# lucastrefezza/quadruplet-sentence-transformer

Hardware: AMD Instinct MI355X
Metric: quadruplets/sec (seq_len=128, all-MiniLM-L6-v2) training step (higher is better)
Workload: dtype bf16; 1 GPU; all-MiniLM-L6-v2 dims (random-init), 64 quadruplets/GPU x 1 GPU, seq_len=128, fwd + gamma-quadruplet loss + bwd + clip + AdamW, dropout 0.1 on hidden states and attention probabilities as the reference's train() mode (BASELINE.json configs[1]); global_batch=64, seq_len=128, parallelism=dp1, precision=bf16 MFMA operands, fp32 accumulate/residual/LN/softmax/loss/optimizer, launch=eager

## Files before the change

### include/qst.h

```cpp
#ifndef QST_H
#define QST_H

#include <stddef.h>
#include <stdint.h>

#ifdef __cplusplus
extern "C" {
#endif

typedef enum {
    QST_OK = 0,
    QST_ERR_BAD_ARG = -1,
    QST_ERR_UNSUPPORTED = -2,
    QST_ERR_WORKSPACE = -3,
    QST_ERR_HIP = -4,
    QST_ERR_NO_DEVICE = -5,
    QST_ERR_COMM = -6,
    QST_ERR_NO_FORWARD = -7
} qst_status;

enum { QST_ARCH_BERT = 0, QST_ARCH_MPNET = 1, QST_ARCH_ROBERTA = 2 };
enum { QST_PREC_BF16 = 0, QST_PREC_BF16X3 = 1, QST_PREC_FP8 = 3, QST_PREC_F16 = 4, QST_PREC_F16W = 5 };
enum { QST_REDUCE_NONE = 0, QST_REDUCE_SUM = 1, QST_REDUCE_MEAN = 2 };

// ... 16 lines not shown

typedef struct qst_encoder qst_encoder;

const char* qst_strerror(int status);
int  qst_last_hip_error(void);
int  qst_version(void);

int64_t qst_arena_elems(const qst_config* cfg);
int     qst_arena_num_segments(const qst_config* cfg);
int     qst_arena_segment(const qst_config* cfg, int idx, const char** name_out, int64_t* offset_out,
                          int64_t* numel_out, int32_t* decay_out, int32_t* gemm_out);
int64_t qst_shadow_elems(const qst_config* cfg);

int64_t qst_shadow8_bytes(const qst_config* cfg);

int  qst_encoder_create(const qst_config* cfg, qst_encoder** out);
void qst_encoder_destroy(qst_encoder* enc);

size_t qst_encoder_saved_bytes(const qst_encoder* enc, int nseq, int L, int training);
size_t qst_encoder_bwd_workspace_bytes(const qst_encoder* enc, int nseq, int L);

int qst_refresh_shadow(const qst_encoder* enc, const float* params, void* shadow_bf16, void* stream);
int qst_refresh_shadow_mx(const qst_encoder* enc, const float* params, void* shadow_mx, void* stream);

int qst_encoder_forward(qst_encoder* enc, const int64_t* ids, const int64_t* mask, const int64_t* type_ids,
                        int nseq, int L, const float* params, const void* shadow_bf16,
                        float* out_emb, float* out_tok, void* saved, size_t saved_bytes, int training,
                        void* stream);

int qst_encoder_set_dropout(qst_encoder* enc, float p_hidden, float p_attn, uint32_t* state_dev);
int qst_dropout_init(uint32_t* state_dev, uint64_t seed, void* stream);
int qst_encoder_set_ffn_chain(qst_encoder* enc, int mask);
int qst_encoder_set_ln_fusion(qst_encoder* enc, int mode);
#define QST_POOL_CLS 1
#define QST_POOL_MAX 2
#define QST_POOL_MEAN 4
#define QST_POOL_MEAN_SQRT 8
#define QST_POOL_WMEAN 16
#define QST_POOL_ALL 31
int qst_encoder_set_pooling(qst_encoder* enc, int mode);
int qst_encoder_embedding_dim(const qst_encoder* enc);
int qst_dropout_advance(uint32_t* state_dev, void* stream);

int qst_encoder_backward(qst_encoder* enc, const int64_t* ids, const int64_t* mask, const int64_t* type_ids,
                         int nseq, int L, const float* params, const void* shadow_bf16,
                         const float* grad_emb, float* grads, void* saved, size_t saved_bytes,
                         void* workspace, size_t workspace_bytes, void* stream);

int qst_encoder_backward_partial(qst_encoder* enc, const int64_t* ids, const int64_t* mask, const int64_t* type_ids,
                                 int nseq, int L, const float* params, const void* shadow_bf16,
                                 const float* grad_emb, float* grads, void* saved, size_t saved_bytes,
                                 void* workspace, size_t workspace_bytes,
                                 int do_head, int layer_hi, int layer_lo, int do_embed, void* stream);

enum { QST_BWD_HEAD = 1, QST_BWD_EMBED = 2, QST_BWD_SKIP_WGRAD = 4, QST_BWD_WGRAD_ONLY = 8 };
int qst_encoder_backward_stage(qst_encoder* enc, const int64_t* ids, const int64_t* mask, const int64_t* type_ids,
                               int nseq, int L, const float* params, const void* shadow_bf16,
                               const float* grad_emb, float* grads, void* saved, size_t saved_bytes,
                               void* workspace, size_t workspace_bytes,
                               int flags, int layer_hi, int layer_lo, void* stream);

int qst_quadruplet_loss(const float* xa, const float* xp, const float* xq, const float* xn,
                        int B, int D, float gamma, float margin_pos_neg, float margin_pos_part,
                        float margin_part_neg, float p, int swap, int reduction,
                        float* out_loss, const float* grad_out,
                        float* grad_a, float* grad_p, float* grad_q, float* grad_n,
// ... 120 lines not shown
```

### quadruplet-sentence-transformer_amd/_lib.py

```python
from __future__ import annotations

import ctypes as C
import os
from typing import Optional

_HERE = os.path.dirname(os.path.abspath(__file__))
LIB_PATH = os.path.join(_HERE, "libqst.so")

c_i64p = C.POINTER(C.c_int64)
c_i32p = C.POINTER(C.c_int32)
c_f32p = C.POINTER(C.c_float)
vp = C.c_void_p


class QstError(RuntimeError):
    pass


class QstConfig(C.Structure):
    _fields_ = [("arch", C.c_int32), ("vocab_size", C.c_int32), ("hidden_size", C.c_int32),
                ("num_layers", C.c_int32), ("num_heads", C.c_int32), ("intermediate_size", C.c_int32),
                ("max_position", C.c_int32), ("type_vocab_size", C.c_int32), ("layer_norm_eps", C.c_float),
                ("normalize", C.c_int32), ("rel_buckets", C.c_int32), ("rel_max_distance", C.c_int32),
                ("pad_token_id", C.c_int32), ("precision", C.c_int32)]
# ... 123 lines not shown
    "qst_gemm_nt8_f8": (C.c_int, [C.POINTER(QstGemmArgs), C.c_int, C.c_int, vp]),
    "qst_gemm8_mode": (C.c_int, [C.c_int]),
    "qst_embed_ln_fwd": (C.c_int, [vp, vp, vp, vp, vp, vp, vp, vp, C.c_float, C.c_int, C.c_int, vp, vp, vp, vp, vp]),
    "qst_embed_ln_fwd_drop": (C.c_int, [vp, vp, vp, vp, vp, vp, vp, vp, C.c_float, C.c_int, C.c_int, vp, vp, vp, vp,
                                        C.POINTER(QstDrop), vp]),
    "qst_ln_fwd_mx": (C.c_int, [vp, vp, vp, C.c_float, C.c_int, C.c_int, vp, vp, vp, vp, vp]),
    "qst_embed_ln_fwd_mx": (C.c_int, [vp, vp, vp, vp, vp, vp, vp, vp, C.c_float, C.c_int, C.c_int, vp, vp, vp, vp, vp]),
    "qst_ln_fwd_mx_train": (C.c_int, [vp, vp, vp, C.c_float, C.c_int, C.c_int, vp, vp, vp, vp, vp, vp, vp]),
    "qst_embed_ln_fwd_mx_train": (C.c_int, [vp, vp, vp, vp, vp, vp, vp, vp, C.c_float, C.c_int, C.c_int, vp, vp, vp, vp, vp, vp,
                                            vp, vp]),
    "qst_ln_fwd": (C.c_int, [vp, vp, vp, C.c_float, C.c_int, C.c_int, vp, vp, vp, vp, vp]),
    "qst_ln_bwd_scratch_bytes": (C.c_size_t, [C.c_int, C.c_int]),
    "qst_ln_bwd_reduce_batch": (C.c_int, [vp, vp]),
    "qst_ln_bwd": (C.c_int, [vp, vp, vp, vp, C.c_int, C.c_int, vp, vp, vp, vp, vp, vp]),
    "qst_ln_bwd_drop": (C.c_int, [vp, vp, vp, vp, C.c_int, C.c_int, vp, vp, vp, vp, vp, C.POINTER(QstDrop), C.POINTER(QstDrop), vp]),
    "qst_embed_bwd": (C.c_int, [vp, vp, vp, vp, C.c_int, C.c_int, C.c_int, C.c_int, vp, vp, vp, vp]),
    "qst_position_ids": (C.c_int, [vp, C.c_int, C.c_int, C.c_int, C.c_int, vp, vp]),
    "qst_forward_prologue": (C.c_int, [vp, C.c_int, C.c_int, C.c_int, C.c_int, vp, vp, vp, vp]),
    "qst_pool_fwd": (C.c_int, [vp, vp, C.c_int, C.c_int, C.c_int, C.c_int, C.c_int, vp, vp, vp, vp]),
    "qst_pool_bwd": (C.c_int, [vp, vp, vp, vp, C.c_int, C.c_int, C.c_int, C.c_int, C.c_int, vp, vp]),
    "qst_attention_fwd": (C.c_int, [vp, vp, vp, C.c_int, C.c_int, C.c_int, C.c_int, vp, vp, vp]),
    "qst_attention_bwd": (C.c_int, [vp, vp, vp, vp, vp, vp, C.c_int, C.c_int, C.c_int, C.c_int, vp, vp, vp, vp]),
    "qst_attention_fwd_ex": (C.c_int, [C.POINTER(QstAttnDesc), vp]),
    "qst_attention_bwd_ex": (C.c_int, [C.POINTER(QstAttnDesc), vp]),
    "qst_dropout_multipliers": (C.c_int, [C.POINTER(QstDrop), C.c_int, C.c_int64, vp, vp]),
    "qst_abi_sizeof": (C.c_int64, [C.c_int]),
    "qst_normalize_rows": (C.c_int, [vp, C.c_int, C.c_int, vp, vp]),
    "qst_cls_head_fwd": (C.c_int, [vp, C.c_int64, C.c_int, C.c_int, vp, vp, vp, vp, C.c_int, C.c_int, C.c_int, vp, vp]),
    "qst_dropout_init": (C.c_int, [vp, C.c_uint64, vp]),
    "qst_dropout_advance": (C.c_int, [vp, vp]),
    "qst_encoder_set_dropout": (C.c_int, [vp, C.c_float, C.c_float, vp]),
    "qst_encoder_set_ffn_chain": (C.c_int, [vp, C.c_int]),
    "qst_encoder_set_ln_fusion": (C.c_int, [vp, C.c_int]),
    "qst_encoder_set_pooling": (C.c_int, [vp, C.c_int]),
    "qst_encoder_embedding_dim": (C.c_int, [vp]),
    "qst_transpose_f32": (C.c_int, [vp, C.c_int, C.c_int, C.c_int, vp, C.c_int, vp]),
    "qst_gelu_f32": (C.c_int, [vp, C.c_int64, vp, vp]),
    "qst_gelu_bwd_f32": (C.c_int, [vp, vp, C.c_int64, vp, vp]),
    "qst_colsum_f32": (C.c_int, [vp, C.c_int, C.c_int, C.c_int, vp, vp]),
    "qst_embed_sum_f32": (C.c_int, [vp, vp, vp, vp, vp, vp, C.c_int, C.c_int, vp, vp]),
    "qst_ln_bwd_f32": (C.c_int, [vp, vp, vp, C.c_float, C.c_int, C.c_int, vp, vp, vp, vp]),
    "qst_attention_bwd_f32": (C.c_int, [vp, vp, vp, vp, vp, C.c_int, C.c_int, C.c_int, C.c_int, vp, vp, vp]),
    "qst_attention_bwd_f32_drop": (C.c_int, [vp, vp, vp, vp, vp, C.c_int, C.c_int, C.c_int, C.c_int, vp, vp, vp, vp]),
    "qst_attention_bwd_x3_scratch_bytes": (C.c_size_t, [C.c_int, C.c_int, C.c_int]),
    "qst_attention_bwd_x3": (C.c_int, [vp, vp, vp, vp, vp, C.c_int, C.c_int, C.c_int, C.c_int, vp, vp, vp, vp, vp]),
    "qst_dropout_apply_f32": (C.c_int, [vp, vp, vp, C.c_int64, vp, vp]),
    "qst_comm_unique_id": (C.c_int, [vp]),
    "qst_comm_init": (C.c_int, [C.c_int, C.c_int, vp, C.POINTER(vp)]),
    "qst_allreduce_bucket": (C.c_int, [vp, vp, C.c_int64, C.c_int, vp]),
    "qst_comm_rank": (C.c_int, [vp]),
    "qst_comm_world": (C.c_int, [vp]),
    "qst_comm_destroy": (None, [vp]),
    "qst_comm_last_error": (C.c_char_p, []),
    "qst_rel_bucket_host": (C.c_int, [C.c_int, C.c_int, C.c_int]),
    "qst_rel_bias_fwd": (C.c_int, [vp, vp, C.c_int, C.c_int, vp, vp]),
    "qst_rel_bias_bwd": (C.c_int, [vp, vp, C.c_int, C.c_int, C.c_int, vp, vp]),
    "qst_rel_pos_fwd": (C.c_int, [vp, vp, C.c_int, C.c_int, vp, vp]),
    "qst_rel_pos_bwd": (C.c_int, [vp, vp, C.c_int, C.c_int, C.c_int, vp, vp]),
    "qst_topk_rows": (C.c_int, [vp, C.c_int64, vp, C.c_int, C.c_int, C.c_int, vp, vp, vp]),
    "qst_topk_merge_rows": (C.c_int, [vp, C.c_int64, C.c_int, C.c_int, C.c_int64, C.c_int64, C.c_int, C.c_float, C.c_int,
                                      vp, vp, vp]),
    "qst_topk_stream_workspace_bytes": (C.c_size_t, [C.c_int, C.c_int, C.c_int]),
    "qst_topk_stream": (C.c_int, [vp, vp, C.c_int, C.c_int, C.c_int, C.c_int, C.c_int, C.c_int, C.c_int64, C.c_int64,
                                  C.c_int, C.c_float, vp, vp, vp, C.c_size_t, vp]),
    "qst_community_workspace_bytes": (C.c_size_t, [C.c_int, C.c_int, C.c_int]),
    "qst_community_count": (C.c_int, [vp, C.c_int, C.c_int, C.c_float, C.c_int, vp, vp, vp, C.c_size_t, vp]),
# ... 70 lines not shown
```

### quadruplet-sentence-transformer_amd/csrc/qst_api.hip

```cpp
#include <math.h>
#include <stdio.h>
#include <string.h>
#include <string>
#include <vector>
#include <mutex>
#include <unordered_map>
#include <algorithm>

#include "qst_common.h"
#include "qst_kernels.h"

static thread_local int g_last_hip_error = 0;
extern "C" int qst_set_hip_error(int code) { g_last_hip_error = code; return code; }
extern "C" int qst_last_hip_error(void) { return g_last_hip_error; }
extern "C" int qst_version(void) { return 114; }

extern "C" const char* qst_strerror(int s) {
    switch (s) {
        case QST_OK: return "ok";
        case QST_ERR_BAD_ARG: return "bad argument (null pointer, non-positive size or bad enum)";
        case QST_ERR_UNSUPPORTED: return "unsupported dimensions for the gfx950 kernels";
        case QST_ERR_WORKSPACE: return "workspace or saved-activation arena too small";
        case QST_ERR_HIP: return "HIP runtime error (see qst_last_hip_error)";
        case QST_ERR_NO_DEVICE: return "no HIP device";
        case QST_ERR_COMM: return "RCCL error (see qst_comm_last_error)";
        case QST_ERR_NO_FORWARD: return "no matching training forward: `saved` is not an activation arena that a training forward of this "
                                        "precision and shape (nseq, L) has filled in this process";
        default: return "unknown qst status";
    }
}

namespace {

constexpr int64_t kAlign = 256;

struct Seg {
    std::string name;
    int64_t off, numel;
    int rows, cols;
    int decay, gemm;
    int64_t shadow_off;
};

struct Layout {
    std::vector<Seg> segs;
    int64_t total = 0, shadow_total = 0;
    int word = -1, pos = -1, type = -1, eg = -1, eb = -1, rel = -1;
    std::vector<int> layer0;
// ... 57 lines not shown
uint64_t g_rec_seq = 0;
void rec_put(const void* saved, uint32_t hidden, uint32_t attn, int kind, int nseq, int L, int pool) {
    std::lock_guard<std::mutex> lk(g_rec_mu);
    g_recs[saved] = FwdRec{hidden, attn, kind, ++g_rec_seq, nseq, L, pool};
    if (g_recs.size() > 4096) {
        std::vector<uint64_t> seqs;
        seqs.reserve(g_recs.size());
        for (const auto& kv : g_recs) seqs.push_back(kv.second.seq);
        std::nth_element(seqs.begin(), seqs.end() - 2048, seqs.end());
        const uint64_t cut = *(seqs.end() - 2048);
        for (auto it = g_recs.begin(); it != g_recs.end();) it = it->second.seq < cut ? g_recs.erase(it) : std::next(it);
    }
}
bool rec_get(const void* saved, int kind, int nseq, int L, FwdRec* out) {
    std::lock_guard<std::mutex> lk(g_rec_mu);
    const auto it = g_recs.find(saved);
    if (it == g_recs.end() || it->second.kind != kind || it->second.nseq != nseq || it->second.L != L) return false;
    *out = it->second;
    return true;
}
}

struct qst_encoder {
    qst_config cfg;
    Layout lay;
    uint8_t* chunk_decay = nullptr;
    int32_t* rel_lut = nullptr;
    int64_t* shadow_tab = nullptr;
    int shadow_nseg = 0, shadow_blocks = 0;
    uint32_t drop_hidden = 0, drop_attn = 0;
    uint32_t* drop_state = nullptr;
    int ffn_chain = 1;
    int ln_fusion = 0;
    int pool = QST_POOL_MEAN;
};

extern "C" int64_t qst_arena_elems(const qst_config* cfg) { return cfg_ok(cfg) ? build_layout(cfg).total : QST_ERR_BAD_ARG; }
extern "C" int64_t qst_shadow_elems(const qst_config* cfg) {
    if (!cfg_ok(cfg)) return QST_ERR_BAD_ARG;
    const int64_t n = build_layout(cfg).shadow_total;
    return cfg->precision == QST_PREC_F16W ? 2 * n : n;
}
extern "C" int64_t qst_shadow8_bytes(const qst_config* cfg) { return cfg_ok(cfg) ? build_layout(cfg).shadow_total : QST_ERR_BAD_ARG; }
extern "C" int qst_arena_num_segments(const qst_config* cfg) { return cfg_ok(cfg) ? (int)build_layout(cfg).segs.size() : QST_ERR_BAD_ARG; }
extern "C" int qst_arena_segment(const qst_config* cfg, int idx, const char** name_out, int64_t* offset_out,
                                 int64_t* numel_out, int32_t* decay_out, int32_t* gemm_out) {
    if (!cfg_ok(cfg)) return QST_ERR_BAD_ARG;
    static thread_local Layout L;
    L = build_layout(cfg);
    if (idx < 0 || idx >= (int)L.segs.size()) return QST_ERR_BAD_ARG;
    const Seg& s = L.segs[idx];
    if (name_out) *name_out = s.name.c_str();
    if (offset_out) *offset_out = s.off;
    if (numel_out) *numel_out = s.numel;
    if (decay_out) *decay_out = s.decay;
    if (gemm_out) *gemm_out = s.gemm;
    return QST_OK;
}

extern "C" int qst_rel_bucket_host(int rel , int num_buckets, int max_distance) {
    int n = -rel;
    const int nb = num_buckets / 2;
    int ret = (n < 0) ? nb : 0;
    n = n < 0 ? -n : n;
    const int max_exact = nb / 2;
    if (n < max_exact) return ret + n;
// ... 168 lines not shown
    return p;
}

struct MxPlan { size_t pos_ids, x[2], xb, xq, xs, qkv, ctx, cq, cs, s, y1, y1b, yq, ys, hq, hs, pooled, rel, argmax, total; };
MxPlan plan_mx(const qst_config& c, int nseq, int L, int pool) {
    MxPlan p;
    const size_t M = (size_t)nseq * L, H = c.hidden_size, I = c.intermediate_size, A = c.num_heads;
    Bump take;
    p.pos_ids = take(M * 4);
    p.x[0] = take(M * H * 4); p.x[1] = take(M * H * 4);
    p.xb = take(M * H * 2); p.xq = take(M * H); p.xs = take(M * H / 32);
    p.qkv = take(M * 3 * H * 2); p.ctx = take(M * H * 2); p.cq = take(M * H); p.cs = take(M * H / 32);
    p.s = take(M * H * 4); p.y1 = take(M * H * 4); p.y1b = take(M * H * 2); p.yq = take(M * H); p.ys = take(M * H / 32);
    p.hq = take(M * I); p.hs = take(M * I / 32);
    p.pooled = take((size_t)nseq * pool_dim(c, pool) * 4);
    p.rel = (c.arch == QST_ARCH_MPNET) ? take(A * (size_t)2 * L * 4) : 0;
    p.argmax = take_argmax(take, c, nseq, pool);
    p.total = take.off;
    return p;
}
struct MxOperands { size_t xq, xs, cq, cs, yq, ys, hq, hs, total; };
MxOperands plan_mx_train_operands(const qst_config& c, int nseq, int L, size_t base) {
    MxOperands t;
    const size_t M = (size_t)nseq * L, H = c.hidden_size, I = c.intermediate_size;
    Bump take{base};
    t.xq = take(M * H); t.xs = take(M * H / 32);
    t.cq = take(M * H); t.cs = take(M * H / 32);
    t.yq = take(M * H); t.ys = take(M * H / 32);
    t.hq = take(M * I); t.hs = take(M * I / 32);
    t.total = take.off;
    return t;
}

struct BwdPlan { size_t dxa, dxb, ds, dsb, dsb1, du, dctx, dqkv, drel, lnred, lnred_stride, delta, total; };
BwdPlan plan_bwd(const qst_config& c, int nseq, int L) {
    BwdPlan p;
    const size_t M = (size_t)nseq * L, H = c.hidden_size, I = c.intermediate_size, A = c.num_heads;
    Bump take;
    p.dxa = take(M * H * 4); p.dxb = take(M * H * 4); p.ds = take(M * H * 4); p.dsb = take(M * H * 2);
    p.dsb1 = take(M * H * 2);
    p.du = take(M * I * 2); p.dctx = take(M * H * 2); p.dqkv = take(M * 3 * H * 2);
    p.drel = (c.arch == QST_ARCH_MPNET) ? take(A * (size_t)2 * L * 4) : 0;
    p.lnred_stride = (qst_ln_bwd_scratch_bytes((int)M, (int)H) + 255) / 256 * 256;
    p.lnred = take(p.lnred_stride * (size_t)(2 * c.num_layers + 1));
    p.delta = take((size_t)nseq * A * L * 4);
    p.total = take.off;
    return p;
}

int shape_ok(const qst_encoder* e, int nseq, int L) {
    if (!e || nseq <= 0 || L <= 0) return QST_ERR_BAD_ARG;
    if (L % 32 != 0 || L > 512) return QST_ERR_UNSUPPORTED;
    if ((int64_t)nseq * L * e->cfg.intermediate_size * 2 >= ((int64_t)1 << 32)) return QST_ERR_UNSUPPORTED;
    if (e->cfg.arch == QST_ARCH_BERT && L > e->cfg.max_position) return QST_ERR_UNSUPPORTED;
    if (e->cfg.arch != QST_ARCH_BERT && L + e->cfg.pad_token_id + 1 > e->cfg.max_position) return QST_ERR_UNSUPPORTED;
    return QST_OK;
}

}

extern "C" int qst_encoder_set_ffn_chain(qst_encoder* e, int mask) {
    if (!e || mask < 0 || mask > 7) return QST_ERR_BAD_ARG;
    e->ffn_chain = mask;
    return QST_OK;
}
extern "C" int qst_encoder_set_ln_fusion(qst_encoder* e, int mode) {
    if (!e || mode < 0 || mode > 2) return QST_ERR_BAD_ARG;
    e->ln_fusion = mode;
    return QST_OK;
}
extern "C" int qst_encoder_set_pooling(qst_encoder* e, int mode) {
    if (!e || mode < 0 || mode > QST_POOL_ALL) return QST_ERR_BAD_ARG;
    e->pool = mode ? mode : QST_POOL_MEAN;
    return QST_OK;
}
extern "C" int qst_encoder_embedding_dim(const qst_encoder* e) {
    return e ? (int)pool_dim(e->cfg, e->pool) : QST_ERR_BAD_ARG;
}
extern "C" int qst_encoder_set_dropout(qst_encoder* e, float p_hidden, float p_attn, uint32_t* state_dev) {
    if (!e || !(p_hidden >= 0.f && p_hidden < 1.f) || !(p_attn >= 0.f && p_attn < 1.f)) return QST_ERR_BAD_ARG;
    if ((p_hidden > 0.f || p_attn > 0.f) && !state_dev) return QST_ERR_BAD_ARG;
    auto thr = [](float p) { const long t = lroundf(p * 65536.f); return (uint32_t)(t > 65535 ? 65535 : t); };
    e->drop_hidden = thr(p_hidden); e->drop_attn = thr(p_attn);
    e->drop_state = (e->drop_hidden || e->drop_attn) ? state_dev : nullptr;
    return QST_OK;
}

extern "C" size_t qst_encoder_saved_bytes(const qst_encoder* e, int nseq, int L, int training) {
    if (shape_ok(e, nseq, L) != QST_OK) return 0;
    const int pool = e->pool;
    if (e->cfg.precision == QST_PREC_BF16X3)
        return training ? plan_x3_train(e->cfg, nseq, L, pool).total : plan_x3(e->cfg, nseq, L, pool).total;
    if (e->cfg.precision == QST_PREC_FP8)
        return training ? plan_mx_train_operands(e->cfg, nseq, L, plan_acts(e->cfg, nseq, L, true, pool).total).total
                        : plan_mx(e->cfg, nseq, L, pool).total;
    return plan_acts(e->cfg, nseq, L, training != 0, pool).total;
}
extern "C" size_t qst_encoder_bwd_workspace_bytes(const qst_encoder* e, int nseq, int L) {
    if (shape_ok(e, nseq, L) != QST_OK) return 0;
    if (e->cfg.precision == QST_PREC_BF16X3) return plan_x3_bwd(e->cfg, nseq, L).total;
    return plan_bwd(e->cfg, nseq, L).total;
}

namespace {

struct OpKernels {
    decltype(&qst_gemm_nt) gemm_nt;
    decltype(&qst_gemm_nt_ln) gemm_nt_ln;
    decltype(&qst_ffn_chain) ffn_chain;
    decltype(&qst_gemm_tn_group) gemm_tn_group;
    decltype(&qst_embed_ln_fwd_drop) embed_ln_fwd_drop;
    decltype(&qst_ln_fwd) ln_fwd;
    decltype(&qst_ln_bwd_drop) ln_bwd_drop;
    decltype(&qst_attention_fwd_ex) attention_fwd_ex;
    decltype(&qst_attention_bwd_ex) attention_bwd_ex;
    decltype(&qst_shadow_all) shadow_all;
    int arena_kind;
};
const OpKernels kOpBf16 = {qst_gemm_nt, qst_gemm_nt_ln, qst_ffn_chain, qst_gemm_tn_group, qst_embed_ln_fwd_drop, qst_ln_fwd,
                           qst_ln_bwd_drop, qst_attention_fwd_ex, qst_attention_bwd_ex, qst_shadow_all, ARENA_BF16};
const OpKernels kOpF16 = {qst_gemm_nt_f16, qst_gemm_nt_ln_f16, qst_ffn_chain_f16, qst_gemm_tn_group_f16,
                          qst_embed_ln_fwd_drop_f16, qst_ln_fwd_f16, qst_ln_bwd_drop_f16, qst_attention_fwd_ex_f16,
                          qst_attention_bwd_ex_f16, qst_shadow_all_f16, ARENA_F16};
const OpKernels& op_kernels(const qst_config& c) {
    return (c.precision == QST_PREC_F16 || c.precision == QST_PREC_F16W) ? kOpF16 : kOpBf16;
}

constexpr int kFuseLnMinRows = 16384;
static bool fuse_ln_rows(int H, int M, int mode) {
    if (!qst_gemm_nt_ln_supported(H) || mode == 2) return false;
    if (mode == 1) return true;
    if (qst_gemm_nt_ln_block_rows(H) == 128) return M >= kFuseLnMinRows;
    return (int64_t)((M + 255) / 256) * (H / 256) >= 512 || (H % 384 == 0 && (int64_t)((M + 127) / 128) * (H / 384) >= 512);
}
// ... 360 lines not shown
        const int b = lay.layer0[l];
        const X3Layer& a = p.layers[l];
        const float* xin = l == 0 ? F(p.x0) : F(p.layers[l - 1].x);
        QST_TRY(qst_ln_bwd_f32(dx, F(a.s2), P(b + LN2_G), eps, M, H, ds, G(b + LN2_G), G(b + LN2_B), st));
        const float* dsm = ds;
        QST_TRY(masked(ds, QST_DROP_SITE_FFN_OUT(l), dctx, &dsm));
        QST_TRY(qst_transpose_f32(P(b + W_2), H, I, I, wT, H, st));
        QST_TRY(nt3(dsm, wT, dbig, I, H, 5, {.aux = F(a.u)}));
        QST_TRY(wgrad(dsm, H, F(a.h), I, b + W_2, b + B_2));
        QST_TRY(dgrad(dbig, I, b + W_1, H, dy, ds));
        QST_TRY(wgrad(dbig, I, F(a.y1), H, b + W_1, b + B_1));
        QST_TRY(qst_ln_bwd_f32(dy, F(a.s1), P(b + LN1_G), eps, M, H, ds, G(b + LN1_G), G(b + LN1_B), st));
        QST_TRY(masked(ds, QST_DROP_SITE_ATTN_OUT(l), dy, &dsm));
        QST_TRY(dgrad(dsm, H, b + W_O, H, dctx, nullptr));
        QST_TRY(wgrad(dsm, H, F(a.ctx), H, b + W_O, b + B_O));
        const QstDrop dp = probs(QST_DROP_SITE_PROBS(l));
        QST_TRY(qst_attention_bwd_x3(F(a.qkv), F(a.ctx), dctx, mask, rel, nseq, L, A, d, dqkv, drel, ws + w.astats, &dp, st));
        QST_TRY(dgrad(dqkv, 3 * H, b + W_QKV, H, dx, ds));
        QST_TRY(wgrad(dqkv, 3 * H, xin, H, b + W_QKV, b + B_QKV));
    }
    if (!(flags & QST_BWD_EMBED)) return QST_OK;
    const QstDrop de = hidden(QST_DROP_SITE_EMBED);
    if (de.state) QST_TRY(qst_dropout_apply_f32(&de, dx, nullptr, (int64_t)M * H, dx, st));
    QST_TRY(qst_ln_bwd_f32(dx, F(p.s0), P(lay.eg), eps, M, H, ds, G(lay.eg), G(lay.eb), st));
    QST_TRY(qst_embed_bwd(ds, ids, type_ids, (const int32_t*)(sv + p.pos_ids), nseq, L, H, c.type_vocab_size,
                          G(lay.word), G(lay.pos), G(lay.type), st));
    if (c.arch == QST_ARCH_MPNET) QST_TRY(qst_rel_bias_bwd(drel, e->rel_lut, c.rel_buckets, A, L, G(lay.rel), st));
    return QST_OK;
}

int Pass::backward_op16(const void* shadow, const float* grad_emb, size_t saved_bytes, size_t workspace_bytes, int flags,
                        int layer_hi, int layer_lo) {
    const ActPlan p = plan_acts(c, nseq, L, true, e->pool);
    const BwdPlan w = plan_bwd(c, nseq, L);
    if (saved_bytes < p.total || workspace_bytes < w.total) return QST_ERR_WORKSPACE;
    const uint16_t* sh = (const uint16_t*)shadow;
    auto WT = [&](int seg) { return sh + lay.segs[seg].shadow_off + qst_align_up(lay.segs[seg].numel, kAlign); };

    float* dxa = (float*)(ws + w.dxa);
    float* dxb = (float*)(ws + w.dxb);
    float* ds = (float*)(ws + w.ds);
    void* dsb = ws + w.dsb;
    void* dsb1 = ws + w.dsb1;
    void* du = ws + w.du;
    void* dctx = ws + w.dctx;
    void* dqkv = ws + w.dqkv;
    QstLnReduceBatch lnb{};
    lnb.H = H;
    lnb.nblocks = (int)(qst_ln_bwd_scratch_bytes(M, H) / ((size_t)2 * H * sizeof(float)));
    const bool fuse_ln = fuse_ln_rows(H, M, e->ln_fusion);
    QST_TRY(backward_dropout(ops.arena_kind, p.dropst));
    const bool fuse_ffn = fuse_ln && !dropping && (e->ffn_chain & 4) && qst_ffn_chain_supported(H, I) != 0;
    const int fused_rows = (M + qst_gemm_nt_ln_block_rows_m(H, M) - 1) / qst_gemm_nt_ln_block_rows_m(H, M);
    auto ln_slot = [&](int slot, float* dg, float* db, int nrows = 0) {
        float* sp = (float*)(ws + w.lnred + (size_t)slot * w.lnred_stride);
        lnb.partials[lnb.count] = sp; lnb.dgamma[lnb.count] = dg; lnb.dbeta[lnb.count] = db;
        lnb.nblocks_each[lnb.count] = nrows;
        ++lnb.count;
        return sp;
    };
    float* drel = nullptr;
    if (c.arch == QST_ARCH_MPNET) {
        drel = (float*)(ws + w.drel);
        rel = F(p.rel);
        if (flags & QST_BWD_HEAD) QST_HIP_CHECK(hipMemsetAsync(drel, 0, (size_t)A * 2 * L * 4, st));
    }
    if (flags & QST_BWD_HEAD) QST_TRY(head_bwd(grad_emb, p.pooled, p.argmax, dxa));
    auto wgrad = [&](int l) -> int {
        const LayerAct& a = p.layers[l];
        const int b = lay.layer0[l];
        const void* xin_b = (l == 0) ? (const void*)(sv + p.x0b) : (const void*)(sv + p.layers[l - 1].xb);
        QstTnGroup grp{};
        grp.nprob = 4;
        grp.splits = 0;
        auto set = [&](int i, const void* dY, int N, const void* X, int K, int wseg, int bseg) {
            QstGemmArgs& q = grp.prob[i];
            q.A = dY; q.B = X; q.C = G(wseg); q.colsum = G(bseg); q.M = M; q.N = N; q.K = K;
            q.lda = N; q.ldb = K; q.ldc = K;
        };
        set(0, dsb, H, sv + a.hact, I, b + W_2, b + B_2);
        set(1, du, I, sv + a.y1b, H, b + W_1, b + B_1);
        set(2, dsb1, H, sv + a.ctx, H, b + W_O, b + B_O);
        set(3, dqkv, 3 * H, xin_b, H, b + W_QKV, b + B_QKV);
        return ops.gemm_tn_group(&grp, st);
    };
    if (flags & QST_BWD_WGRAD_ONLY) return wgrad(layer_lo);
    for (int l = layer_hi - 1; l >= layer_lo; --l) {
        const LayerAct& a = p.layers[l];
        const int b = lay.layer0[l];
        if (!fuse_ln || l == c.num_layers - 1)
            QST_TRY(ops.ln_bwd_drop(dxa, sv + a.xh2, F(a.rs2), P(b + LN2_G), M, H, ds, dsb, nullptr, nullptr,
                                    ln_slot(2 * l + 1, G(b + LN2_G), G(b + LN2_B)), nullptr,
                                    active(hidden(QST_DROP_SITE_FFN_OUT(l))), st));
        if (!fuse_ffn) QST_TRY(nt(dsb, WT(b + W_2), du, I, H, QST_EPI_GELU_BWD, {.aux = sv + a.u}));
        const float* ds1 = ds;
        const QstDrop d1 = hidden(QST_DROP_SITE_ATTN_OUT(l));
        if (fuse_ffn) {
            QST_TRY(ffn({.A = dsb, .B1 = WT(b + W_2), .B2 = WT(b + W_1), .resid = ds, .aux = sv + a.u, .save_h = du, .C = dxb,
                         .C2 = dsb1},
                        1, {.gamma = P(b + LN1_G), .xhat = sv + a.xh1, .rstd = F(a.rs1),
                            .partials = ln_slot(2 * l, G(b + LN1_G), G(b + LN1_B), fused_rows)}));
            ds1 = dxb;
        } else if (fuse_ln) {
            QST_TRY(nt_ln(du, WT(b + W_1), dxb, I, 1, {.C2 = dsb1, .resid = ds, .drop = d1, .drop_where = 2},
                          {.gamma = P(b + LN1_G), .xhat = sv + a.xh1, .rstd = F(a.rs1),
                           .partials = ln_slot(2 * l, G(b + LN1_G), G(b + LN1_B), fused_rows)}));
            ds1 = dxb;
        } else {
            QST_TRY(nt(du, WT(b + W_1), dxb, H, I, QST_EPI_F32_RESID, {.resid = ds}));
            QST_TRY(ops.ln_bwd_drop(dxb, sv + a.xh1, F(a.rs1), P(b + LN1_G), M, H, ds, dsb1, nullptr, nullptr,
                                    ln_slot(2 * l, G(b + LN1_G), G(b + LN1_B)), nullptr, active(d1), st));
        }
        QST_TRY(nt(dsb1, WT(b + W_O), dctx, H, H, QST_EPI_BF16));
        QstAttnDesc q = attn(l, sv + a.qkv, sv + a.ctx, F(a.lse));
        q.dctx = dctx; q.dqkv = dqkv; q.drel = drel; q.delta_scratch = (float*)(ws + w.delta);
        QST_TRY(ops.attention_bwd_ex(&q, st));
        if (!(flags & QST_BWD_SKIP_WGRAD)) QST_TRY(wgrad(l));
        if (fuse_ln && l > 0) {
            const LayerAct& lo = p.layers[l - 1];
            const int bl = lay.layer0[l - 1];
            QST_TRY(nt_ln(dqkv, WT(b + W_QKV), ds, 3 * H, 1,
                          {.C2 = dsb, .resid = ds1, .drop = hidden(QST_DROP_SITE_FFN_OUT(l - 1)), .drop_where = 2},
                          {.gamma = P(bl + LN2_G), .xhat = sv + lo.xh2, .rstd = F(lo.rs2),
                           .partials = ln_slot(2 * (l - 1) + 1, G(bl + LN2_G), G(bl + LN2_B), fused_rows)}));
        } else if (fuse_ln) {
            QST_TRY(nt_ln(dqkv, WT(b + W_QKV), ds, 3 * H, 1, {.resid = ds1, .drop = hidden(QST_DROP_SITE_EMBED), .drop_where = 3},
                          {.gamma = P(lay.eg), .xhat = sv + p.xh0, .rstd = F(p.rs0),
                           .partials = ln_slot(2 * c.num_layers, G(lay.eg), G(lay.eb), fused_rows)}));
        } else {
            QST_TRY(nt(dqkv, WT(b + W_QKV), dxa, H, 3 * H, QST_EPI_F32_RESID, {.resid = ds1}));
        }
    }
    const bool do_embed = (flags & QST_BWD_EMBED) != 0;
    if (do_embed && !fuse_ln)
        QST_TRY(ops.ln_bwd_drop(dxa, sv + p.xh0, F(p.rs0), P(lay.eg), M, H, ds, nullptr, nullptr, nullptr,
                                ln_slot(2 * c.num_layers, G(lay.eg), G(lay.eb)), active(hidden(QST_DROP_SITE_EMBED)), nullptr, st));
    if (lnb.count > 0) {
        if (lnb.count > QST_LN_BATCH_MAX) return QST_ERR_UNSUPPORTED;
        QST_TRY(qst_ln_bwd_reduce_batch(&lnb, st));
    }
    if (!do_embed) return QST_OK;
    QST_TRY(qst_embed_bwd(ds, ids, type_ids, (const int32_t*)(sv + p.pos_ids), nseq, L, H, c.type_vocab_size,
                          G(lay.word), G(lay.pos), G(lay.type), st));
    if (c.arch == QST_ARCH_MPNET) QST_TRY(qst_rel_pos_bwd(drel, e->rel_lut, c.rel_buckets, A, L, G(lay.rel), st));
    return QST_OK;
}

}

extern "C" int qst_refresh_shadow(const qst_encoder* e, const float* params, void* shadow, void* stream) {
    if (!e || !params || !shadow) return QST_ERR_BAD_ARG;
    if (e->cfg.precision == QST_PREC_F16W)
        return qst_shadow_all_split_f16(params, shadow, (uint16_t*)shadow + e->lay.shadow_total, e->shadow_tab, e->shadow_nseg,
                                        e->shadow_blocks, stream);
    return op_kernels(e->cfg).shadow_all(params, shadow, e->shadow_tab, e->shadow_nseg, e->shadow_blocks, stream);
// ... 144 lines not shown
```

### quadruplet-sentence-transformer_amd/encoder.py

```python
from __future__ import annotations

from dataclasses import dataclass
from typing import Dict, Optional, Tuple

import numpy as np
import torch

from . import _lib
from .config import EncoderConfig, build_layout, hf_param_views, pooling_mask


def _round_up(n: int, m: int) -> int:
    return (n + m - 1) // m * m


@dataclass(frozen=True)
class _Precision:
    name: str
    aliases: tuple
    code: int
    shadow_size: Optional[str] = None
    shadow_dtype: Optional[torch.dtype] = None
    refresh: Optional[str] = None
    bwd_shadow: str = "bf16"
# ... 28 lines not shown
    stale: bool = True


def _stale_flag(name: str) -> property:
    def get(self) -> bool:
        rec = self._live.get(name)
        return True if rec is None else rec.stale

    def put(self, stale) -> None:
        rec = self._live.get(name)
        if rec is not None:
            rec.stale = bool(stale)
    return property(get, put)


class HipEncoder:
    def __init__(self, cfg: EncoderConfig, device: Optional[torch.device] = None, precision: int = 0):
        self.cfg = cfg
        self.lib = _lib.load()
        if not torch.cuda.is_available():
            raise _lib.QstError("HipEncoder needs a HIP device; there is no CPU fallback")
        self.device = torch.device(device) if device is not None else torch.device("cuda", torch.cuda.current_device())
        torch.cuda.set_device(self.device)
        self.ccfg = _lib.make_config(cfg, precision)
        self.segments, self.total = build_layout(cfg)
        n = self.lib.qst_arena_elems(self.ccfg)
        if n != self.total:
            raise _lib.QstError(f"arena layout mismatch: python {self.total} vs libqst {n}")
        self.pool_mode = pooling_mask(cfg.pooling)
        self.dropout = None
        self.dropout_step = 0
        self.drop_state = None
        self.ln_fusion = 0
        self._live: Dict[str, _Live] = {}
        self._record("bf16")
        self.emb_dim = self.lib.qst_encoder_embedding_dim(self.handle)
        if self.emb_dim != cfg.embedding_dim:
            raise _lib.QstError(f"embedding width mismatch: python {cfg.embedding_dim} vs libqst {self.emb_dim}")
        self.amp_scaler: Optional[torch.Tensor] = None
        self._step2_dev: Optional[torch.Tensor] = None
        self.params = torch.zeros(self.total, dtype=torch.float32, device=self.device)
        self.grads: Optional[torch.Tensor] = None
        self.exp_avg: Optional[torch.Tensor] = None
        self.exp_avg_sq: Optional[torch.Tensor] = None
        self._arenas: Dict[str, torch.Tensor] = {}
        self._scratch = torch.zeros(2048, dtype=torch.float32, device=self.device)
        self._step_dev: Optional[torch.Tensor] = None
        self.grad_norm = torch.zeros(1, dtype=torch.float32, device=self.device)
        self.opt_step = 0

    def _create(self, ccfg, what: str):
        h = _lib.vp()
        _lib.check(self.lib.qst_encoder_create(ccfg, h), what)
        try:
            if self.pool_mode != pooling_mask("mean"):
                _lib.check(self.lib.qst_encoder_set_pooling(h, self.pool_mode), "qst_encoder_set_pooling")
            if self.dropout is not None:
                _lib.check(self.lib.qst_encoder_set_dropout(h, self.dropout[0], self.dropout[1], self.drop_state.data_ptr()),
                           "qst_encoder_set_dropout")
            if self.ln_fusion:
                _lib.check(self.lib.qst_encoder_set_ln_fusion(h, self.ln_fusion), "qst_encoder_set_ln_fusion")
        except Exception:
            self.lib.qst_encoder_destroy(h)
            raise
        return h

    def _record(self, precision) -> _Live:
        spec = _precision(precision)
        rec = self._live.get(spec.name)
        if rec is None:
            ccfg = self.ccfg if spec.name == "bf16" else _lib.make_config(self.cfg, spec.code)
            h = self._create(ccfg, f"qst_encoder_create({spec.name})")
            try:
                shadow = None if spec.shadow_size is None else torch.zeros(
                    getattr(self.lib, spec.shadow_size)(ccfg), dtype=spec.shadow_dtype, device=self.device)
            except Exception:
                self.lib.qst_encoder_destroy(h)
                raise
            rec = self._live[spec.name] = _Live(spec, h, shadow)
        return rec

    def _handle_for(self, precision):
        return self._record(precision).handle

    @property
    def handle(self):
        return self._live["bf16"].handle

    shadow_stale = _stale_flag("bf16")
    shadow_mx_stale = _stale_flag("fp8")
    shadow_f16_stale = _stale_flag("f16")
    shadow_f16w_stale = _stale_flag("f16w")

    def __del__(self):
# ... 28 lines not shown
            n = int(np.prod(shape))
            out[name] = self.grads[s.offset + off: s.offset + off + n].view(*shape)
        return out

    def ensure_train_state(self) -> None:
        if self.grads is None:
            self.grads = torch.zeros_like(self.params)
        if self.exp_avg is None:
            self.exp_avg = torch.zeros_like(self.params)
            self.exp_avg_sq = torch.zeros_like(self.params)

    def set_dropout(self, p_hidden: float = 0.0, p_attn: float = 0.0, seed: int = 0) -> None:
        if not (0.0 <= p_hidden < 1.0 and 0.0 <= p_attn < 1.0):
            raise ValueError("dropout probabilities must be in [0, 1)")
        on = p_hidden > 0.0 or p_attn > 0.0
        if on:
            if self.drop_state is None:
                self.drop_state = torch.zeros(4, dtype=torch.int32, device=self.device)
            _lib.check(self.lib.qst_dropout_init(self.drop_state.data_ptr(), int(seed) & 0xFFFFFFFFFFFFFFFF,
                                                 _lib.current_stream_ptr()), "qst_dropout_init")
        for rec in self._live.values():
            _lib.check(self.lib.qst_encoder_set_dropout(rec.handle, float(p_hidden), float(p_attn),
                                                        self.drop_state.data_ptr() if on else None), "qst_encoder_set_dropout")
        self.dropout = (float(p_hidden), float(p_attn), int(seed)) if on else None
        self.dropout_step = 0

    def set_ffn_chain(self, mask: int) -> None:
        _lib.check(self.lib.qst_encoder_set_ffn_chain(self.handle, int(mask)), "qst_encoder_set_ffn_chain")

    def set_ln_fusion(self, mode: int) -> None:
        for rec in self._live.values():
            _lib.check(self.lib.qst_encoder_set_ln_fusion(rec.handle, int(mode)), "qst_encoder_set_ln_fusion")
        self.ln_fusion = int(mode)

    def set_dropout_step(self, step: int) -> None:
        if self.dropout is not None:
            self.drop_state[2] = int(step)
            self.dropout_step = int(step)

    def refresh_shadow(self, precision="bf16") -> None:
        rec = self._record(precision)
        if rec.shadow is None:
            raise ValueError(f"precision {rec.spec.name!r} has no operand shadow")
        _lib.check(getattr(self.lib, rec.spec.refresh)(rec.handle, self.params.data_ptr(), rec.shadow.data_ptr(),
                                                       _lib.current_stream_ptr()), f"{rec.spec.refresh}({rec.spec.name})")
        rec.stale = False

    def mark_stale(self, keep=None) -> None:
        fresh = None if keep is None else _precision(keep).name
        for name, rec in self._live.items():
            rec.stale = name != fresh

    @staticmethod
    def pad_inputs(ids: torch.Tensor, mask: torch.Tensor, type_ids: Optional[torch.Tensor], pad_id: int
                   ) -> Tuple[torch.Tensor, torch.Tensor, Optional[torch.Tensor], int]:
        n, L = ids.shape
        Lp = _round_up(L, 32)
        if Lp != L:
            ids = torch.nn.functional.pad(ids, (0, Lp - L), value=pad_id)
            mask = torch.nn.functional.pad(mask, (0, Lp - L), value=0)
            if type_ids is not None:
                type_ids = torch.nn.functional.pad(type_ids, (0, Lp - L), value=0)
        return ids.contiguous(), mask.contiguous(), None if type_ids is None else type_ids.contiguous(), L

    def _arena(self, name: str, nbytes: int) -> torch.Tensor:
        buf = self._arenas.get(name)
# ... 138 lines not shown
```

Baseline: 14180 quadruplets/s.

## Batch weight-gradient GEMMs of two adjacent layers into one grouped launch

Adds a wgrad-pairing mode that double-buffers the per-layer backward gradient buffers (dsb, dsb1, du, dqkv). This lets the weight-gradient GEMMs of two consecutive layers be issued as one grouped TN launch with eight problems instead of two launches with four. A default rule turns pairing on when one layer yields 32–63 output tiles of size 192 and the row count is large, which is meant to fill more compute units per launch. The cost is extra workspace for the second buffer set and a delayed wgrad for the upper layer of each pair.

```diff
diff --git a/include/qst.h b/include/qst.h
--- a/include/qst.h
+++ b/include/qst.h
@@ -72,6 +72,9 @@
 int qst_dropout_init(uint32_t* state_dev, uint64_t seed, void* stream);
 int qst_encoder_set_ffn_chain(qst_encoder* enc, int mask);
 int qst_encoder_set_ln_fusion(qst_encoder* enc, int mode);
+int qst_encoder_set_wgrad_pairs(qst_encoder* enc, int mode);
+int qst_wgrad_pairs_rule(const qst_config* cfg, int M);
+int qst_wgrad_tiles(const qst_config* cfg, int M, int layers);
 #define QST_POOL_CLS 1
 #define QST_POOL_MAX 2
 #define QST_POOL_MEAN 4
diff --git a/quadruplet-sentence-transformer_amd/_lib.py b/quadruplet-sentence-transformer_amd/_lib.py
--- a/quadruplet-sentence-transformer_amd/_lib.py
+++ b/quadruplet-sentence-transformer_amd/_lib.py
@@ -179,6 +179,9 @@
     "qst_encoder_set_dropout": (C.c_int, [vp, C.c_float, C.c_float, vp]),
     "qst_encoder_set_ffn_chain": (C.c_int, [vp, C.c_int]),
     "qst_encoder_set_ln_fusion": (C.c_int, [vp, C.c_int]),
+    "qst_encoder_set_wgrad_pairs": (C.c_int, [vp, C.c_int]),
+    "qst_wgrad_pairs_rule": (C.c_int, [C.POINTER(QstConfig), C.c_int]),
+    "qst_wgrad_tiles": (C.c_int, [C.POINTER(QstConfig), C.c_int, C.c_int]),
     "qst_encoder_set_pooling": (C.c_int, [vp, C.c_int]),
     "qst_encoder_embedding_dim": (C.c_int, [vp]),
     "qst_transpose_f32": (C.c_int, [vp, C.c_int, C.c_int, C.c_int, vp, C.c_int, vp]),
diff --git a/quadruplet-sentence-transformer_amd/csrc/qst_api.hip b/quadruplet-sentence-transformer_amd/csrc/qst_api.hip
--- a/quadruplet-sentence-transformer_amd/csrc/qst_api.hip
+++ b/quadruplet-sentence-transformer_amd/csrc/qst_api.hip
@@ -13,7 +13,7 @@
 static thread_local int g_last_hip_error = 0;
 extern "C" int qst_set_hip_error(int code) { g_last_hip_error = code; return code; }
 extern "C" int qst_last_hip_error(void) { return g_last_hip_error; }
-extern "C" int qst_version(void) { return 114; }
+extern "C" int qst_version(void) { return 115; }
 
 extern "C" const char* qst_strerror(int s) {
     switch (s) {
@@ -137,6 +137,7 @@
     uint32_t* drop_state = nullptr;
     int ffn_chain = 1;
     int ln_fusion = 0;
+    int wgrad_pairs = 0;
     int pool = QST_POOL_MEAN;
 };
 
@@ -371,20 +372,53 @@
     return t;
 }
 
-struct BwdPlan { size_t dxa, dxb, ds, dsb, dsb1, du, dctx, dqkv, drel, lnred, lnred_stride, delta, total; };
-BwdPlan plan_bwd(const qst_config& c, int nseq, int L) {
+struct BwdPlan { size_t dxa, dxb, ds, dsb[2], dsb1[2], du[2], dctx, dqkv[2], drel, lnred, lnred_stride, delta, total; };
+BwdPlan plan_bwd(const qst_config& c, int nseq, int L, bool pair) {
     BwdPlan p;
     const size_t M = (size_t)nseq * L, H = c.hidden_size, I = c.intermediate_size, A = c.num_heads;
     Bump take;
-    p.dxa = take(M * H * 4); p.dxb = take(M * H * 4); p.ds = take(M * H * 4); p.dsb = take(M * H * 2);
-    p.dsb1 = take(M * H * 2);
-    p.du = take(M * I * 2); p.dctx = take(M * H * 2); p.dqkv = take(M * 3 * H * 2);
+    p.dxa = take(M * H * 4); p.dxb = take(M * H * 4); p.ds = take(M * H * 4); p.dsb[0] = take(M * H * 2);
+    p.dsb1[0] = take(M * H * 2);
+    p.du[0] = take(M * I * 2); p.dctx = take(M * H * 2); p.dqkv[0] = take(M * 3 * H * 2);
     p.drel = (c.arch == QST_ARCH_MPNET) ? take(A * (size_t)2 * L * 4) : 0;
     p.lnred_stride = (qst_ln_bwd_scratch_bytes((int)M, (int)H) + 255) / 256 * 256;
     p.lnred = take(p.lnred_stride * (size_t)(2 * c.num_layers + 1));
     p.delta = take((size_t)nseq * A * L * 4);
+    p.dsb[1] = pair ? take(M * H * 2) : p.dsb[0];
+    p.dsb1[1] = pair ? take(M * H * 2) : p.dsb1[0];
+    p.du[1] = pair ? take(M * I * 2) : p.du[0];
+    p.dqkv[1] = pair ? take(M * 3 * H * 2) : p.dqkv[0];
     p.total = take.off;
     return p;
+}
+
+void wgrad_shapes(QstTnGroup& g, int at, int M, int H, int I) {
+    const int nk[4][2] = {{H, I}, {I, H}, {H, H}, {3 * H, H}};
+    for (int i = 0; i < 4; ++i) {
+        QstGemmArgs& q = g.prob[at + i];
+        q.M = M; q.N = nk[i][0]; q.K = nk[i][1];
+        q.lda = q.N; q.ldb = q.K; q.ldc = q.K;
+    }
+}
+constexpr int kTnTile = 192;
+int wgrad_tiles(const qst_config& c, int M, int layers) {
+    QstTnGroup g{};
+    g.nprob = 4 * layers;
+    for (int k = 0; k < layers; ++k) wgrad_shapes(g, 4 * k, M, c.hidden_size, c.intermediate_size);
+    int tiles = 0;
+    for (int i = 0; i < g.nprob; ++i)
+        tiles += ((g.prob[i].N + kTnTile - 1) / kTnTile) * ((g.prob[i].K + kTnTile - 1) / kTnTile);
+    return tiles;
+}
+static_assert(QST_TN_MAX_PROB >= 8, "a launch takes the weight gradients of two layers");
+
+constexpr int kWgradPairMinRows = 8192;
+bool wgrad_pair_rule(const qst_config& c, int M) {
+    const int tiles = wgrad_tiles(c, M, 1);
+    return c.num_layers >= 2 && M >= kWgradPairMinRows && tiles >= 32 && tiles < 2 * 32;
+}
+bool wgrad_pairing(const qst_config& c, int M, int mode) {
+    return c.num_layers >= 2 && (mode == 2 || (mode == 0 && wgrad_pair_rule(c, M)));
 }
 
 int shape_ok(const qst_encoder* e, int nseq, int L) {
@@ -407,6 +441,19 @@
     if (!e || mode < 0 || mode > 2) return QST_ERR_BAD_ARG;
     e->ln_fusion = mode;
     return QST_OK;
+}
+extern "C" int qst_encoder_set_wgrad_pairs(qst_encoder* e, int mode) {
+    if (!e || mode < 0 || mode > 2) return QST_ERR_BAD_ARG;
+    e->wgrad_pairs = mode;
+    return QST_OK;
+}
+extern "C" int qst_wgrad_pairs_rule(const qst_config* cfg, int M) {
+    if (!cfg_ok(cfg) || M <= 0) return QST_ERR_BAD_ARG;
+    return wgrad_pair_rule(*cfg, M) ? 1 : 0;
+}
+extern "C" int qst_wgrad_tiles(const qst_config* cfg, int M, int layers) {
+    if (!cfg_ok(cfg) || M <= 0 || layers < 1 || layers > 2) return QST_ERR_BAD_ARG;
+    return wgrad_tiles(*cfg, M, layers);
 }
 extern "C" int qst_encoder_set_pooling(qst_encoder* e, int mode) {
     if (!e || mode < 0 || mode > QST_POOL_ALL) return QST_ERR_BAD_ARG;
@@ -438,7 +485,7 @@
 extern "C" size_t qst_encoder_bwd_workspace_bytes(const qst_encoder* e, int nseq, int L) {
     if (shape_ok(e, nseq, L) != QST_OK) return 0;
     if (e->cfg.precision == QST_PREC_BF16X3) return plan_x3_bwd(e->cfg, nseq, L).total;
-    return plan_bwd(e->cfg, nseq, L).total;
+    return plan_bwd(e->cfg, nseq, L, wgrad_pairing(e->cfg, nseq * L, e->wgrad_pairs)).total;
 }
 
 namespace {
@@ -865,19 +912,17 @@
 int Pass::backward_op16(const void* shadow, const float* grad_emb, size_t saved_bytes, size_t workspace_bytes, int flags,
                         int layer_hi, int layer_lo) {
     const ActPlan p = plan_acts(c, nseq, L, true, e->pool);
-    const BwdPlan w = plan_bwd(c, nseq, L);
+    const BwdPlan w = plan_bwd(c, nseq, L, wgrad_pairing(c, M, e->wgrad_pairs));
     if (saved_bytes < p.total || workspace_bytes < w.total) return QST_ERR_WORKSPACE;
+    const bool pairing = w.dsb[1] != w.dsb[0] && layer_hi - layer_lo >= 2 && !(flags & (QST_BWD_SKIP_WGRAD | QST_BWD_WGRAD_ONLY));
     const uint16_t* sh = (const uint16_t*)shadow;
     auto WT = [&](int seg) { return sh + lay.segs[seg].shadow_off + qst_align_up(lay.segs[seg].numel, kAlign); };
 
     float* dxa = (float*)(ws + w.dxa);
     float* dxb = (float*)(ws + w.dxb);
     float* ds = (float*)(ws + w.ds);
-    void* dsb = ws + w.dsb;
-    void* dsb1 = ws + w.dsb1;
-    void* du = ws + w.du;
     void* dctx = ws + w.dctx;
-    void* dqkv = ws + w.dqkv;
+    auto set_of = [&](int l) { return pairing && l >= layer_lo ? (layer_hi - 1 - l) & 1 : 0; };
     QstLnReduceBatch lnb{};
     lnb.H = H;
     lnb.nblocks = (int)(qst_ln_bwd_scratch_bytes(M, H) / ((size_t)2 * H * sizeof(float)));
@@ -899,28 +944,33 @@
         if (flags & QST_BWD_HEAD) QST_HIP_CHECK(hipMemsetAsync(drel, 0, (size_t)A * 2 * L * 4, st));
     }
     if (flags & QST_BWD_HEAD) QST_TRY(head_bwd(grad_emb, p.pooled, p.argmax, dxa));
-    auto wgrad = [&](int l) -> int {
-        const LayerAct& a = p.layers[l];
-        const int b = lay.layer0[l];
-        const void* xin_b = (l == 0) ? (const void*)(sv + p.x0b) : (const void*)(sv + p.layers[l - 1].xb);
+    auto wgrad = [&](int l_up, int layers) -> int {
         QstTnGroup grp{};
-        grp.nprob = 4;
+        grp.nprob = 4 * layers;
         grp.splits = 0;
-        auto set = [&](int i, const void* dY, int N, const void* X, int K, int wseg, int bseg) {
-            QstGemmArgs& q = grp.prob[i];
-            q.A = dY; q.B = X; q.C = G(wseg); q.colsum = G(bseg); q.M = M; q.N = N; q.K = K;
-            q.lda = N; q.ldb = K; q.ldc = K;
-        };
-        set(0, dsb, H, sv + a.hact, I, b + W_2, b + B_2);
-        set(1, du, I, sv + a.y1b, H, b + W_1, b + B_1);
-        set(2, dsb1, H, sv + a.ctx, H, b + W_O, b + B_O);
-        set(3, dqkv, 3 * H, xin_b, H, b + W_QKV, b + B_QKV);
+        for (int k = 0; k < layers; ++k) {
+            const int l = l_up - k, s = set_of(l);
+            const LayerAct& a = p.layers[l];
+            const int b = lay.layer0[l];
+            const void* xin_b = (l == 0) ? (const void*)(sv + p.x0b) : (const void*)(sv + p.layers[l - 1].xb);
+            wgrad_shapes(grp, 4 * k, M, H, I);
+            auto set = [&](int i, const void* dY, const void* X, int wseg, int bseg) {
+                QstGemmArgs& q = grp.prob[4 * k + i];
+                q.A = dY; q.B = X; q.C = G(wseg); q.colsum = G(bseg);
+            };
+            set(0, ws + w.dsb[s], sv + a.hact, b + W_2, b + B_2);
+            set(1, ws + w.du[s], sv + a.y1b, b + W_1, b + B_1);
+            set(2, ws + w.dsb1[s], sv + a.ctx, b + W_O, b + B_O);
+            set(3, ws + w.dqkv[s], xin_b, b + W_QKV, b + B_QKV);
+        }
         return ops.gemm_tn_group(&grp, st);
     };
-    if (flags & QST_BWD_WGRAD_ONLY) return wgrad(layer_lo);
+    if (flags & QST_BWD_WGRAD_ONLY) return wgrad(layer_lo, 1);
     for (int l = layer_hi - 1; l >= layer_lo; --l) {
         const LayerAct& a = p.layers[l];
         const int b = lay.layer0[l];
+        const int s = set_of(l);
+        void *dsb = ws + w.dsb[s], *dsb1 = ws + w.dsb1[s], *du = ws + w.du[s], *dqkv = ws + w.dqkv[s];
         if (!fuse_ln || l == c.num_layers - 1)
             QST_TRY(ops.ln_bwd_drop(dxa, sv + a.xh2, F(a.rs2), P(b + LN2_G), M, H, ds, dsb, nullptr, nullptr,
                                     ln_slot(2 * l + 1, G(b + LN2_G), G(b + LN2_B)), nullptr,
@@ -948,12 +998,16 @@
         QstAttnDesc q = attn(l, sv + a.qkv, sv + a.ctx, F(a.lse));
         q.dctx = dctx; q.dqkv = dqkv; q.drel = drel; q.delta_scratch = (float*)(ws + w.delta);
         QST_TRY(ops.attention_bwd_ex(&q, st));
-        if (!(flags & QST_BWD_SKIP_WGRAD)) QST_TRY(wgrad(l));
+        if (!pairing) {
+            if (!(flags & QST_BWD_SKIP_WGRAD)) QST_TRY(wgrad(l, 1));
+        } else if (((l - layer_lo) & 1) == 0) {
+            QST_TRY(wgrad(l + 1 < layer_hi ? l + 1 : l, l + 1 < layer_hi ? 2 : 1));
+        }
         if (fuse_ln && l > 0) {
             const LayerAct& lo = p.layers[l - 1];
             const int bl = lay.layer0[l - 1];
             QST_TRY(nt_ln(dqkv, WT(b + W_QKV), ds, 3 * H, 1,
-                          {.C2 = dsb, .resid = ds1, .drop = hidden(QST_DROP_SITE_FFN_OUT(l - 1)), .drop_where = 2},
+                          {.C2 = ws + w.dsb[set_of(l - 1)], .resid = ds1, .drop = hidden(QST_DROP_SITE_FFN_OUT(l - 1)), .drop_where = 2},
                           {.gamma = P(bl + LN2_G), .xhat = sv + lo.xh2, .rstd = F(lo.rs2),
                            .partials = ln_slot(2 * (l - 1) + 1, G(bl + LN2_G), G(bl + LN2_B), fused_rows)}));
         } else if (fuse_ln) {
diff --git a/quadruplet-sentence-transformer_amd/encoder.py b/quadruplet-sentence-transformer_amd/encoder.py
--- a/quadruplet-sentence-transformer_amd/encoder.py
+++ b/quadruplet-sentence-transformer_amd/encoder.py
@@ -84,6 +84,7 @@
         self.dropout_step = 0
         self.drop_state = None
         self.ln_fusion = 0
+        self.wgrad_pairs = 0
         self._live: Dict[str, _Live] = {}
         self._record("bf16")
         self.emb_dim = self.lib.qst_encoder_embedding_dim(self.handle)
@@ -112,6 +113,8 @@
                            "qst_encoder_set_dropout")
             if self.ln_fusion:
                 _lib.check(self.lib.qst_encoder_set_ln_fusion(h, self.ln_fusion), "qst_encoder_set_ln_fusion")
+            if self.wgrad_pairs:
+                _lib.check(self.lib.qst_encoder_set_wgrad_pairs(h, self.wgrad_pairs), "qst_encoder_set_wgrad_pairs")
         except Exception:
             self.lib.qst_encoder_destroy(h)
             raise
@@ -206,6 +209,11 @@
         for rec in self._live.values():
             _lib.check(self.lib.qst_encoder_set_ln_fusion(rec.handle, int(mode)), "qst_encoder_set_ln_fusion")
         self.ln_fusion = int(mode)
+
+    def set_wgrad_pairs(self, mode: int) -> None:
+        for rec in self._live.values():
+            _lib.check(self.lib.qst_encoder_set_wgrad_pairs(rec.handle, int(mode)), "qst_encoder_set_wgrad_pairs")
+        self.wgrad_pairs = int(mode)
 
     def set_dropout_step(self, step: int) -> None:
         if self.dropout is not None:
```

New measurement: 14400 quadruplets/s (median of 6 runs). 1.5% higher.
